# devincody/DSAbeamformer

Measured on AMD Instinct MI355X. Metric: beam-blocks/sec (256 beams x 256 freq x N_TIME), higher is better.
Workload: dtype int8 (int32 accumulate, fp32 detect)

## Files before the change

dsabeamformer_amd/api.py:

```python
from __future__ import annotations

import ctypes as C

from ._lib import BF_CAL_FULL, BF_CAL_PHASE, BfCalOptions, BfCondOptions, BfConfig, BfSkOptions, DsabfError, BfSpsCandidate, BfSpsPeak, BfSpsStat, check, load


def debug_config(**over) -> BfConfig:
    cfg = BfConfig()
    check(load().bf_config_default(C.byref(cfg), 1))
    for k, v in over.items():
        setattr(cfg, k, v)
    return cfg


def production_config(**over) -> BfConfig:
    cfg = BfConfig()
    check(load().bf_config_default(C.byref(cfg), 0))
    for k, v in over.items():
        setattr(cfg, k, v)
    return cfg


def launch_plan(cfg: BfConfig, paired: bool, n_units: int = 1, n_cus: int = 256) -> dict:
    g, b, l = C.c_int(), C.c_int(), C.c_int()
# ... 180 lines not shown
        check(self._lib.bf_stream_sync(self._h, stream_idx))

    def timer_start(self) -> None:
        check(self._lib.bf_timer_start(self._h))

    def timer_stop(self) -> float:
        ms = C.c_float()
        check(self._lib.bf_timer_stop(self._h, C.byref(ms)))
        return ms.value

    def mfma_peak(self, d_operands, operand_bytes: int, d_scratch, scratch_bytes: int, iters: int, stream) -> float:
        ops = C.c_double()
        check(self._lib.bf_mfma_peak_device(self._h, _ptr(d_operands), operand_bytes, _ptr(d_scratch), scratch_bytes, iters,
                                            C.byref(ops), C.c_void_p(stream)))
        return ops.value

    def gather_relayout(self, d_stage, d_full, rows_held: int, world: int, row_floats: int, skip_rank: int, stream: int = 0) -> None:
        check(self._lib.bf_gather_relayout_device(self._h, _ptr(d_stage), _ptr(d_full), rows_held, world, row_floats, skip_rank,
                                                  C.c_void_p(stream)))

    def set_switch(self, name: str, value: int) -> None:
        check(self._lib.bf_set_switch(self._h, name.encode(), int(value)))

    def counter(self, name: str) -> int:
        v = C.c_uint64()
        check(self._lib.bf_get_counter(self._h, name.encode(), C.byref(v)))
        return int(v.value)

    def kernel_info(self, n_units: int = 1) -> dict:
        g, b, l, v = C.c_int(), C.c_int(), C.c_int(), C.c_int()
        check(self._lib.bf_kernel_info(self._h, n_units, C.byref(g), C.byref(b), C.byref(l), C.byref(v)))
        name = C.create_string_buffer(160)
        check(self._lib.bf_kernel_name(self._h, name, 160))
        return {"kernel": name.value.decode(), "grid": g.value, "block": b.value, "lds_bytes": l.value,
                "vgprs": v.value}

    def variant_key(self, write_c: bool = False) -> str:
        buf = C.create_string_buffer(120)
        check(self._lib.bf_handle_variant_key(self._h, int(write_c), buf, 120))
        return buf.value.decode()


class DmStream(_Owner):
    _ptr_attr, _destroy = "_s", "bf_dm_stream_destroy"

    def __init__(self, bf: Beamformer, delays, n_freq_total: int, max_rows_per_push: int):
        import numpy as np

        self._lib = load()
        self._s = C.c_void_p()
        d = np.ascontiguousarray(delays, np.int32)
        assert d.ndim == 2 and d.shape[1] == n_freq_total
        self.n_dm, self.n_beams, self._bf = d.shape[0], bf.cfg.n_beams, bf
        check(self._lib.bf_dm_stream_create(bf._h, _ptr(d), d.shape[0], n_freq_total, max_rows_per_push, C.byref(self._s)))

    @property
    def max_delay(self) -> int:
        return self._lib.bf_dm_stream_max_delay(self._s)

    def push(self, d_rows, n_rows: int, host_out=None, stream: int = 0):
        first, n = C.c_uint64(), C.c_int()
        check(self._lib.bf_dm_stream_push(self._s, _ptr(d_rows), n_rows, _ptr(host_out), C.byref(first), C.byref(n), C.c_void_p(stream)))
        return int(first.value), int(n.value)

    def reserve(self, n_rows: int, stream: int = 0) -> int:
        p = C.c_void_p()
        check(self._lib.bf_dm_stream_reserve(self._s, n_rows, C.byref(p), C.c_void_p(stream)))
        return p.value or 0
# ... 342 lines not shown
```

dsabeamformer_amd/csrc/bf_bench_abi.cpp:

```cpp
#include "../../include/dsabf_bench.h"

#include <cstring>

#include "bf_runtime_internal.h"

extern "C" {

int bf_mfma_peak_device(bf_handle* h, const void* d_operands, size_t operand_bytes, void* d_scratch, size_t scratch_bytes, int iters,
                        double* ops, void* hip_stream)
{
    if (!h || !d_operands || !d_scratch) return fail(BF_ERR_INVALID, "NULL argument");
    if (operand_bytes < dsabf::kMfmaPeakSrcBytes || scratch_bytes < dsabf::kMfmaPeakSinkBytes || ((uintptr_t)d_operands & 15) || iters <= 0)
        return fail(BF_ERR_INVALID, "need >= %zu operand bytes (16-byte aligned), >= %zu scratch bytes, iters > 0",
                    dsabf::kMfmaPeakSrcBytes, dsabf::kMfmaPeakSinkBytes);
    ON_DEVICE(h);
    HIP_TRY(dsabf::launch_mfma_peak(d_operands, d_scratch, iters, h->n_cus, ops, as_stream(hip_stream)));
    return BF_OK;
}

int bf_gather_relayout_device(bf_handle* h, const float* d_stage, float* d_full, size_t rows_held, int world, size_t row_floats,
                              int skip_rank, void* hip_stream)
{
    if (!h || !d_stage || !d_full) return fail(BF_ERR_INVALID, "NULL argument");
    if (world < 1 || row_floats % 4 || ((uintptr_t)d_stage & 15) || ((uintptr_t)d_full & 15))
// ... 20 lines not shown
            FLUSH_UNITS(h);
            h->geom.fold = false;
        }
    } else if (!strcmp(name, "dm_wide")) {
        h->geom.dm_wide = value != 0;
    } else if (!strcmp(name, "coalesce")) {
        FLUSH_UNITS(h);
        h->coalesce = value != 0;
    } else if (!strcmp(name, "paired")) {
        h->force_general = value == 0;
    } else if (!strcmp(name, "fold")) {
        h->no_fold = value == 0;
    } else if (!strcmp(name, "dm_ring")) {
        h->dm_ring = value != 0;
    } else if (!strcmp(name, "cal_resident")) {
        h->cal_resident = value != 0;
    } else {
        return fail(BF_ERR_INVALID, "unknown switch \"%s\" (tsplit, rtw_kout, lds_pad, dm_wide, dm_ring, paired, fold, coalesce, cal_resident)", name);
    }
    return BF_OK;
}

int bf_get_counter(const bf_handle* h, const char* name, uint64_t* value)
{
    if (!h || !name || !value) return fail(BF_ERR_INVALID, "NULL argument");
    if (!strcmp(name, "fused_launches"))
        *value = h->n_fused_launches;
    else if (!strcmp(name, "queued_units"))
        *value = h->pending.size();
    else if (!strcmp(name, "dm_ring_stages")) {
        uint64_t n = 0;
        for (const bf_stage* s : h->stages) n += s->ring ? 1 : 0;
        *value = n;
    } else
        return fail(BF_ERR_INVALID, "unknown counter \"%s\" (fused_launches, queued_units, dm_ring_stages)", name);
    return BF_OK;
}

int bf_kernel_info(const bf_handle* h, int n_units, int* grid, int* block, int* lds_bytes, int* vgprs)
{
    if (!h) return fail(BF_ERR_INVALID, "handle is NULL");
    const dsabf::LaunchShape ls = dsabf::fused_launch_shape(h->geom, n_units > 0 ? n_units : 1, h->n_cus);
    if (grid) *grid = ls.grid;
    if (block) *block = ls.block;
    if (lds_bytes) *lds_bytes = ls.lds_bytes;
    if (vgprs) *vgprs = dsabf::fused_vgprs(h->geom);
    return BF_OK;
}

int bf_launch_plan(const bf_config* cfg, int paired, int n_units, int n_cus, int* grid, int* block, int* lds_bytes, char* name,
                   size_t name_len)
{
    dsabf::Geometry g{};
    if (int rc = supported_geom(cfg, g)) return rc;
    if (n_units <= 0 || n_cus <= 0) return fail(BF_ERR_INVALID, "need n_units > 0 and n_cus > 0");
    g.paired = paired && dsabf::pairing_supported(g);
    const dsabf::LaunchShape ls = dsabf::fused_launch_shape(g, n_units, n_cus);
    if (grid) *grid = ls.grid;
    if (block) *block = ls.block;
    if (lds_bytes) *lds_bytes = ls.lds_bytes;
    if (name && name_len) dsabf::fused_kernel_name(g, name, name_len);
    return BF_OK;
}

int bf_rtw_plan(const bf_config* cfg, int n_units, int n_cus, int* windows_per_stream, int* chunks_total)
{
    dsabf::Geometry g{};
    if (int rc = supported_geom(cfg, g)) return rc;
// ... 33 lines not shown
```

dsabeamformer_amd/csrc/bf_fused16.hpp:

```cpp
#pragma once
#include "bf_kernels.h"

#include <hip/hip_runtime.h>

#include <atomic>
#include <type_traits>

#ifndef DSABF_CLOCKPROBE
#define DSABF_CLOCKPROBE 0
#endif

namespace dsabf {

typedef int v4i __attribute__((ext_vector_type(4)));
typedef float v2f __attribute__((ext_vector_type(2)));
typedef float v4f __attribute__((ext_vector_type(4)));

constexpr int kDetCanonical = 0;
constexpr int kDetFast = 1;
constexpr int kDetContracted = 2;

constexpr int kAntK1P16 = -1;
constexpr int kAntK1P4 = -2;
constexpr int kAntK2P16 = -3;
// ... 76 lines not shown
{
    constexpr int LR = NIPO >= 32 ? 32 : 16;
    return chunk ^ ((((row >> 1) & 1) | (((row / LR) & 3) << 1)) ^ ((row & 1) << 2));
}

constexpr int kWaves16 = 4;
constexpr int kThreads16 = 64 * kWaves16;
constexpr int kWavesWide16 = 8;
constexpr int kColTiles16 = 4;
constexpr int kColTilesWide16 = 8;

template <int AIN>
constexpr int ant_ksteps()
{
    if (AIN > 0) return (AIN + 63) / 64;
    return (AIN == kAntK4P16 || AIN == kAntK4P4) ? 4 : (AIN == kAntK3P16 || AIN == kAntK3P4) ? 3 : (AIN == kAntK2P16 || AIN == kAntK2P4) ? 2 : 1;
}
template <int AIN>
constexpr bool ant_two_ksteps() { return ant_ksteps<AIN>() == 2; }
template <int AIN>
constexpr bool ant_deep() { return ant_ksteps<AIN>() > 2; }

template <int AIN, int NIPO, bool WRITE_C, int NS = kColTiles16>
constexpr int fused_min_waves()
{
    if (NS == 8 || ant_ksteps<AIN>() >= 2) return 2;
    if (AIN == kAntK1P16 && (NIPO == 8 || NIPO == 16 || NIPO == 32) && !WRITE_C) return 4;
    return 3;
}

template <int AIN, int NIPO, bool WRITE_C, int MODE = kDetCanonical, bool PAIRED = false, int WAVES = kWaves16, int NS = kColTiles16>
__global__ __launch_bounds__(64 * WAVES, (fused_min_waves<AIN, NIPO, WRITE_C, NS>())) void fused16_kernel(FusedArgs a)
{
    constexpr bool FOLD = false;
#include "bf_fused16_body.inc"
}

template <int NIPO>
struct FoldShape {
    static constexpr int AIN = kAntK1P16, WAVES = kWaves16, NS = kColTiles16;
    static constexpr bool WRITE_C = false, PAIRED = false;
};
template <int NIPO, int MODE>
__global__ __launch_bounds__(kThreads16, (fused_min_waves<kAntK1P16, NIPO, false>())) void fused16_fold_kernel(FusedArgs a)
{
    constexpr int AIN = FoldShape<NIPO>::AIN, WAVES = FoldShape<NIPO>::WAVES, NS = FoldShape<NIPO>::NS;
    constexpr bool WRITE_C = FoldShape<NIPO>::WRITE_C, PAIRED = FoldShape<NIPO>::PAIRED, FOLD = true;
#include "bf_fused16_body.inc"
}

template <int AIN, int NIPO, bool WRITE_C, int MODE, bool PAIRED, int WAVES, int NS>
hipError_t launch_fused16_t(const FusedArgs& args, const LaunchShape& ls, hipStream_t s)
{
    auto kern = fused16_kernel<AIN, NIPO, WRITE_C, MODE, PAIRED, WAVES, NS>;
    if (ls.block != 64 * WAVES || (args.interleave && args.interleave != (PAIRED ? NS / 2 : NS))) return hipErrorInvalidValue;
    if (ls.lds_bytes > 48 * 1024) {
        static std::atomic<unsigned> done_mask{0};
        int dev = 0;
        (void)hipGetDevice(&dev);
        const unsigned bit = 1u << (dev & 31);
        if (dev >= 32 || !(done_mask.load(std::memory_order_acquire) & bit)) {
            hipError_t e = hipFuncSetAttribute(reinterpret_cast<const void*>(kern), hipFuncAttributeMaxDynamicSharedMemorySize,
                                               ls.lds_bytes);
            if (e != hipSuccess) return e;
            done_mask.fetch_or(bit, std::memory_order_release);
        }
    }
    (void)hipGetLastError();
    hipLaunchKernelGGL(kern, dim3(ls.grid), dim3(ls.block), ls.lds_bytes, s, args);
    return hipGetLastError();
}

template <int NIPO, int MODE>
hipError_t launch_fused16_fold_t(const FusedArgs& args, const LaunchShape& ls, hipStream_t s)
{
    if (ls.block != kThreads16 || args.n_ant != 64 || (args.interleave && args.interleave != kColTiles16) || ls.lds_bytes > 48 * 1024)
        return hipErrorInvalidValue;
    (void)hipGetLastError();
    hipLaunchKernelGGL((fused16_fold_kernel<NIPO, MODE>), dim3(ls.grid), dim3(ls.block), ls.lds_bytes, s, args);
    return hipGetLastError();
}

using fused_launch_fn = hipError_t (*)(const FusedArgs&, const LaunchShape&, hipStream_t);
struct FusedVariant {
    const void* fn = nullptr;
    fused_launch_fn launch = nullptr;
    int ain = 0, nipo = 0, write_c = 0, mode = 0, paired = 0, waves = 0, ns = 0;
    int fold = 0;
};

template <int AIN, int NIPO, bool WRITE_C, int MODE, bool PAIRED, int WAVES, int NS = kColTiles16>
FusedVariant make_variant()
{
    return FusedVariant{reinterpret_cast<const void*>(fused16_kernel<AIN, NIPO, WRITE_C, MODE, PAIRED, WAVES, NS>),
                        launch_fused16_t<AIN, NIPO, WRITE_C, MODE, PAIRED, WAVES, NS>, AIN, NIPO, WRITE_C, MODE, PAIRED, WAVES, NS};
}

template <int AIN, int NIPO, int WAVES>
FusedVariant fused16_variant_nipo(bool write_c, int mode, bool paired)
{
    if (write_c) {
        if constexpr (WAVES == kWaves16) return make_variant<AIN, NIPO, true, kDetCanonical, false, WAVES>();
        return FusedVariant{};
    }
    if constexpr (NIPO >= 16 || NIPO == 0) {
        if (mode == kDetFast)
            return paired ? make_variant<AIN, NIPO, false, kDetFast, true, WAVES>() : make_variant<AIN, NIPO, false, kDetFast, false, WAVES>();
    }
    if (mode == kDetContracted)
        return paired ? make_variant<AIN, NIPO, false, kDetContracted, true, WAVES>()
                      : make_variant<AIN, NIPO, false, kDetContracted, false, WAVES>();
    return paired ? make_variant<AIN, NIPO, false, kDetCanonical, true, WAVES>() : make_variant<AIN, NIPO, false, kDetCanonical, false, WAVES>();
}

template <int AIN>
// ... 68 lines not shown
        if (mode == kDetFast) return make_variant<AIN, NIPO, false, kDetFast, true, kWavesWide16, 4>();
        if (mode == kDetContracted) return make_variant<AIN, NIPO, false, kDetContracted, true, kWavesWide16, 4>();
        return make_variant<AIN, NIPO, false, kDetCanonical, true, kWavesWide16, 4>();
    }
    if (mode == kDetFast) return make_variant<AIN, NIPO, false, kDetFast, false, kWavesWide16, 2>();
    if (mode == kDetContracted) return make_variant<AIN, NIPO, false, kDetContracted, false, kWavesWide16, 2>();
    return make_variant<AIN, NIPO, false, kDetCanonical, false, kWavesWide16, 2>();
}
template <int AIN>
FusedVariant fused16_variant_deep(int n_ipo, int mode, bool paired, int ns)
{
    static_assert(ant_deep<AIN>(), "three or four k-steps");
    switch (n_ipo) {
        case 16: return fused16_variant_deep_nipo<AIN, 16>(mode, paired, ns);
        case 32: return fused16_variant_deep_nipo<AIN, 32>(mode, paired, ns);
        case 64:
            if constexpr (AIN == kAntK3P4 || AIN == kAntK4P4) return FusedVariant{};
            else return fused16_variant_deep_nipo<AIN, 64>(mode, paired, ns);
        default: return FusedVariant{};
    }
}
FusedVariant fused16_variant_k4p16(int n_ipo, int mode, bool paired, int ns);
FusedVariant fused16_variant_k3p16(int n_ipo, int mode, bool paired, int ns);
FusedVariant fused16_variant_k4p4(int n_ipo, int mode, bool paired, int ns);
FusedVariant fused16_variant_k3p4(int n_ipo, int mode, bool paired, int ns);

template <int NIPO, int MODE>
FusedVariant make_fold_variant()
{
    return FusedVariant{reinterpret_cast<const void*>(fused16_fold_kernel<NIPO, MODE>), launch_fused16_fold_t<NIPO, MODE>, kAntK1P16, NIPO, 0, MODE,
                        0, kWaves16, kColTiles16, 1};
}
FusedVariant fused16_variant_k1p16_fold(int n_ipo, int mode);

FusedVariant fused16_variant_a100(int n_ipo, bool write_c, int mode, bool paired);
FusedVariant fused16_variant_k1p16(int n_ipo, bool write_c, int mode, bool paired);
FusedVariant fused16_variant_k1p4(int n_ipo, bool write_c, int mode, bool paired);
FusedVariant fused16_variant_k2p16(int n_ipo, bool write_c, int mode, bool paired);
FusedVariant fused16_variant_k2p4(int n_ipo, bool write_c, int mode, bool paired);
FusedVariant fused16_variant_a100_w8(int n_ipo, int mode);
FusedVariant fused16_variant_k2p16_w8(int n_ipo, int mode);
FusedVariant fused16_variant_k2p4_w8(int n_ipo, int mode);
FusedVariant fused16_variant_a100_w8p(int n_ipo, int mode);
FusedVariant fused16_variant_k2p16_w8p(int n_ipo, int mode);
FusedVariant fused16_variant_k2p4_w8p(int n_ipo, int mode);
FusedVariant fused16_variant_a100_s8(int n_ipo, int mode);
FusedVariant fused16_variant_k2p16_s8(int n_ipo, int mode);
FusedVariant fused16_variant_k2p4_s8(int n_ipo, int mode);

}
```

dsabeamformer_amd/csrc/bf_fused16_body.inc:

```
    constexpr int THREADS = 64 * WAVES;
    constexpr bool FAST = MODE == kDetFast;
    constexpr bool CONTRACTED = MODE == kDetContracted;
    constexpr bool RTW = NIPO == 0;
    constexpr int MAPN = RTW ? 32 : NIPO;
    static_assert(!FAST || ((NIPO >= 16 || RTW) && !WRITE_C), "the fast detect exists for n_ipo >= 16 only");
    static_assert(!RTW || (WAVES == kWaves16 && NS == kColTiles16 && !ant_deep<AIN>()), "run-time windows: the plain launch shape");
    static_assert(!(PAIRED && WRITE_C), "the stage-parity path always runs the general kernel");
    static_assert(AIN >= kAntK3P4 && AIN != 0 && (AIN < 0 || AIN % 4 == 0) && AIN <= 256, "antenna class");
    static_assert(!ant_deep<AIN>() || (WAVES == 8 && NIPO >= 16 && !WRITE_C), "deep classes: 8 waves, long windows");
    static_assert(!FOLD || (AIN == kAntK1P16 && NIPO >= 16 && !WRITE_C && !PAIRED && WAVES == kWaves16 && NS == kColTiles16),
                  "antenna fold: 64 antennas in 16-byte pieces, long compile-time windows, general tiles on the plain launch shape");
    constexpr bool OFFSET_NIB = ant_deep<AIN>();
    constexpr float kA = FOLD ? kAlpha8 : OFFSET_NIB ? kAlpha : kAlpha16;
    constexpr float kNKA = FOLD ? kNegMagicAlpha8 : OFFSET_NIB ? kNegMagicAlpha : kNegMagicAlpha16;
    constexpr bool RT = AIN < 0;
    constexpr int RB = 128;
    constexpr int KS = ant_ksteps<AIN>();
    constexpr int PLANE = kRowsPerChunk * RB;
    constexpr int BUF = KS * PLANE;
    constexpr bool DW = RT ? (AIN == kAntK1P4 || AIN == kAntK2P4 || AIN == kAntK3P4 || AIN == kAntK4P4) : (AIN % 16) != 0;
    constexpr int PB = DW ? 4 : 16;
    constexpr int AMAX = RT ? 64 * KS : AIN;
    const int A = FOLD ? 64 : RT ? a.n_ant : AIN;
    const int PPR = A / PB;
    const int TOTALP = kRowsPerChunk * PPR;
    constexpr int TOTALP_MAX = kRowsPerChunk * (AMAX / PB);
    constexpr int NT = PAIRED ? NS / 2 : NS;
    constexpr bool LONG = NIPO >= 16;
    constexpr int L = LONG ? NIPO : 16;
    constexpr int LR = (NIPO >= 32 || RTW) ? 32 : 16;
    constexpr int CPG = L > 32 ? L / 32 : 1;
    constexpr int PPT = (TOTALP_MAX + THREADS - 1) / THREADS;
    using stage_t = std::conditional_t<DW, int, v4i>;

    extern __shared__ __attribute__((aligned(16))) char smem[];

    const int tid = threadIdx.x;
    const int lane = tid & 63;
    const int wave = __builtin_amdgcn_readfirstlane(tid >> 6);
    const int g4 = lane >> 4;
    const int c16 = lane & 15;

    int f, bg, ts;
    decode_block(a, f, bg, ts);
// ... 58 lines not shown
            sacc += __shfl_xor(sacc, 32);
            return sacc;
        };
#pragma unroll
        for (int t = 0; t < NT; t++) {
            int s0, s1;
            if constexpr (PAIRED) {
                s0 = (int)kMagicBits - 8 * colsum(bw[t][0]);
                s1 = -8 * colsum(bw[t][1]);
            } else {
                const int wr = colsum(bw[t][0]), nwi = colsum(bw[t][1]), wi = colsum(bw[t][2]);
                s0 = (int)kMagicBits - 8 * (wr + nwi);
                s1 = (int)kMagicBits - 8 * (wi + wr);
            }
            sd[t][0] = v4i{s0, s0, s0, s0};
            sd[t][1] = v4i{s1, s1, s1, s1};
            asm volatile("" : "+v"(sd[t][0]), "+v"(sd[t][1]));
        }
    }

    auto run_sample0 = [&](int c, int run) -> unsigned {
        if constexpr (RTW)
            return (4u * (unsigned)(c / cpg_rt) + (unsigned)run) * (unsigned)a.rt_Ls + 32u * (unsigned)(c % cpg_rt);
        else if constexpr (NIPO >= 32)
            return (4u * (unsigned)(c / CPG) + (unsigned)run) * (unsigned)L + 32u * (unsigned)(c % CPG);
        else
            return (unsigned)c * 128u + 16u * (unsigned)run;
    };
    stage_t stage[PPT];
    constexpr unsigned SPAN = (NIPO == 64) ? 256u : 128u;
    const bool fast_addr = !RTW && ((unsigned)a.T % SPAN) == 0;
    [[maybe_unused]] unsigned lane_off64[NIPO == 64 ? PPT : 1];
    int lds_re[PPT];
#pragma unroll
    for (int k = 0; k < PPT; k++) {
        int row, pi;
        if constexpr (FOLD) {
            row = tid >> 1;
            pi = k == 0 ? (tid & 1) : 3 - (tid & 1);
        } else {
            const int pc = tid + k * THREADS;
            row = (pc / PPR) % kRowsPerChunk, pi = pc % PPR;
        }
        if constexpr (NIPO == 64) lane_off64[k] = (unsigned)((row / LR) * L + (row % LR)) * A + pi * PB;
        const int blk = DW ? pi / 4 : pi;
        const int h = blk / 4, kp = blk % 4, sub = DW ? 4 * (pi % 4) : 0;
        lds_re[k] = h * PLANE + row * RB + 16 * swz16<MAPN>(kp + 4 * (h & 1), row) + sub;
    }
    auto lane_off = [&](int k) -> unsigned {
        if constexpr (NIPO == 64)
            return lane_off64[k];
        else if constexpr (FOLD)
            return (unsigned)(64 * (tid >> 1) + 16 * (k == 0 ? (tid & 1) : 3 - (tid & 1)));
        else
            return (unsigned)PB * (unsigned)(tid + k * THREADS);
    };
    auto piece_live = [&](int k) { return (!RT && TOTALP_MAX % THREADS == 0) || (tid + k * THREADS < TOTALP); };
    int ld_span = -1;
    unsigned ld_u = 0, ld_t0 = 0;
    auto load_chunk = [&](int c) {
        if (fast_addr) {
            const int span = (NIPO == 64) ? c / 2 : c;
            if (ld_span < 0) {
                const unsigned s_c = (unsigned)span * SPAN;
                ld_u = a.t_shift >= 0 ? (s_c >> a.t_shift) : (s_c / (unsigned)a.T);
                ld_t0 = s_c - ld_u * (unsigned)a.T;
                ld_span = span;
            }
            while (ld_span < span) {
                ld_t0 += SPAN;
                if (ld_t0 >= (unsigned)a.T) {
                    ld_t0 = 0;
                    ld_u++;
                }
                ld_span++;
            }
            const bool valid = (unsigned)span * SPAN < a.S;
            const unsigned half = (NIPO == 64) ? 32u * (unsigned)(c & 1) : 0u;
            const uint8_t* base = a.in + ((size_t)((size_t)ld_u * a.n_freq + f) * a.T + ld_t0 + half) * A;
#pragma unroll
            for (int k = 0; k < PPT; k++) {
                stage[k] = stage_t{};
                if (valid && piece_live(k)) stage[k] = *reinterpret_cast<const stage_t*>(base + lane_off(k));
            }
            return;
        }
#pragma unroll
        for (int k = 0; k < PPT; k++) {
            int row, pi;
            if constexpr (FOLD) {
                row = tid >> 1;
                pi = k == 0 ? (tid & 1) : 3 - (tid & 1);
            } else {
                const int pc = tid + k * THREADS;
                row = (pc / PPR) % kRowsPerChunk, pi = pc % PPR;
            }
            const unsigned s0 = run_sample0(c, row / LR) + (unsigned)(row % LR);
            stage[k] = stage_t{};
            bool row_ok = s0 < a.S;
            if constexpr (RTW) row_ok = row_ok && 32u * (unsigned)(c % cpg_rt) + (unsigned)(row % LR) < (unsigned)a.rt_Ls;
            if (row_ok && piece_live(k)) {
                const unsigned u = a.t_shift >= 0 ? (s0 >> a.t_shift) : (s0 / (unsigned)a.T);
                const unsigned t = s0 - u * (unsigned)a.T;
                stage[k] = *reinterpret_cast<const stage_t*>(a.in + ((size_t)((size_t)u * a.n_freq + f) * a.T + t) * A + pi * PB);
            }
        }
    };
    auto write_chunk = [&](char* buf) {
        if constexpr (FOLD) {
            constexpr unsigned M = 0x78787878u, H = 0x80808080u;
            v4i sr, si, dr, di;
#pragma unroll
            for (int d = 0; d < 4; d++) {
                const unsigned ta = (unsigned)stage[0][d] ^ 0x88888888u;
                const unsigned tb = __builtin_bswap32((unsigned)stage[PPT - 1][3 - d]) ^ 0x88888888u;
                const unsigned ra = (ta >> 1) & M, ia = (ta << 3) & M, rb = (tb >> 1) & M, ib = (tb << 3) & M;
                sr[d] = (int)((ra + rb) ^ H);
                si[d] = (int)((ia + ib) ^ H);
                dr[d] = (int)(((ra | H) - rb) ^ H);
                di[d] = (int)(((ia | H) - ib) ^ H);
            }
            *reinterpret_cast<v4i*>(buf + lds_re[0]) = sr;
            *reinterpret_cast<v4i*>(buf + (lds_re[0] ^ 32)) = di;
            *reinterpret_cast<v4i*>(buf + (lds_re[0] ^ 64)) = dr;
            *reinterpret_cast<v4i*>(buf + (lds_re[0] ^ 96)) = si;
            return;
        }
#pragma unroll
        for (int k = 0; k < PPT; k++) {
            if (!piece_live(k)) continue;
            if constexpr (DW) {
                const unsigned w = (unsigned)stage[k];
                if constexpr (OFFSET_NIB) {
                    const unsigned x = w ^ 0x88888888u;
                    *reinterpret_cast<int*>(buf + lds_re[k]) = (int)((x >> 4) & 0x0F0F0F0Fu);
                    *reinterpret_cast<int*>(buf + (lds_re[k] ^ 64)) = (int)(x & 0x0F0F0F0Fu);
                } else {
                    *reinterpret_cast<int*>(buf + lds_re[k]) = (int)(w & 0xF0F0F0F0u);
                    *reinterpret_cast<int*>(buf + (lds_re[k] ^ 64)) = (int)((w << 4) & 0xF0F0F0F0u);
                }
            } else {
                v4i re, im;
#pragma unroll
// ... 25 lines not shown
    for (int gi = 0; gi < PEND; gi++) pend_chunk[gi] = -1;
    auto store_slots = [&](float* row, const float (&x)[NS]) {
        if (a.interleave) {
            if constexpr (PAIRED && NS == 2) {
                row[slot_beam[0]] = x[0];
                row[slot_beam[1]] = x[1];
            } else if constexpr (PAIRED && NS == 4) {
                __builtin_nontemporal_store(v2f{x[0], x[2]}, reinterpret_cast<v2f*>(row + slot_beam[0]));
                __builtin_nontemporal_store(v2f{x[3], x[1]}, reinterpret_cast<v2f*>(row + slot_beam[3]));
            } else if constexpr (PAIRED) {
                __builtin_nontemporal_store(v4f{x[0], x[2], x[4], x[6]}, reinterpret_cast<v4f*>(row + slot_beam[0]));
                __builtin_nontemporal_store(v4f{x[7], x[5], x[3], x[1]}, reinterpret_cast<v4f*>(row + slot_beam[7]));
            } else if constexpr (NS == 2) {
                __builtin_nontemporal_store(v2f{x[0], x[1]}, reinterpret_cast<v2f*>(row + slot_beam[0]));
            } else {
#pragma unroll
                for (int q = 0; q < NS; q += 4)
                    __builtin_nontemporal_store(v4f{x[q], x[q + 1], x[q + 2], x[q + 3]}, reinterpret_cast<v4f*>(row + slot_beam[q]));
            }
        } else {
#pragma unroll
            for (int sl = 0; sl < NS; sl++)
                if (slot_beam[sl] < a.n_beams) row[slot_beam[sl]] = x[sl];
        }
    };
    auto flush_pending = [&]() {
        if constexpr (LONG && !WRITE_C) {
#pragma unroll
            for (int gi = 0; gi < PEND; gi++) {
                if (pend_chunk[gi] >= 0 && wave_active) {
                    const unsigned grp = (NIPO >= 32) ? (unsigned)(pend_chunk[gi] / CPG) : (2u * pend_chunk[gi] + gi);
                    float* ub = a.out + ((size_t)(4u * grp) * FB + (size_t)f * a.n_beams);
                    const unsigned o = 4u * grp + (unsigned)g4;
                    if (o * (unsigned)L < a.S) store_slots(ub + (size_t)g4 * FB, pend[gi]);
                }
                pend_chunk[gi] = -1;
            }
        }
    };

    if (c_begin >= c_end) return;
#if DSABF_CLOCKPROBE
    const unsigned long long probe_t0 = __builtin_amdgcn_s_memtime(), probe_r0 = __builtin_amdgcn_s_memrealtime();
#endif

    load_chunk(c_begin);
    write_chunk(smem);
    if (c_begin + 1 < c_end) load_chunk(c_begin + 1);
    __syncthreads();

    const bool stage_only = FOLD && !wave_active;
    if (stage_only)
        for (int c = c_begin; c < c_end; c++) {
            if (c + 1 < c_end) write_chunk(smem + ((c - c_begin + 1) & 1) * BUF);
            if (c + 2 < c_end) load_chunk(c + 2);
            __syncthreads();
        }
    for (int c = stage_only ? c_end : c_begin; c < c_end; c++) {
        char* cur = smem + ((c - c_begin) & 1) * BUF;
        char* nxt = smem + ((c - c_begin + 1) & 1) * BUF;
        if (!FOLD && !wave_active) {
            if (c + 1 < c_end) write_chunk(nxt);
            if (c + 2 < c_end) load_chunk(c + 2);
        } else {
            [[maybe_unused]] float ov[2][NS];
            [[maybe_unused]] bool rt_st[4] = {false, false, false, false}, rt_en[4] = {false, false, false, false};
            [[maybe_unused]] unsigned rt_o[4] = {0, 0, 0, 0};
            [[maybe_unused]] float rt_x[4][NS];
            [[maybe_unused]] int rt_m = 0;
            [[maybe_unused]] unsigned rt_oq = 0;
            if constexpr (RTW) {
                const unsigned p0 = 32u * (unsigned)(c % cpg_rt);
                rt_m = (int)(p0 % (unsigned)a.rt_L);
                rt_oq = p0 / (unsigned)a.rt_L;
            }
            auto detect = [&](const int t8, const v4f fr, const v4f fi, const int sl) {
                const int gi = (NIPO >= 32) ? 0 : (t8 >> 2);
                const int q4 = (NIPO >= 32) ? (32 * (c % CPG) + 4 * t8) : 4 * (t8 & 3);
                const unsigned grp = (NIPO >= 32) ? (unsigned)(c / CPG) : (2u * (unsigned)c + gi);
                const unsigned o = 4u * grp + (unsigned)g4;
                const int beam = slot_beam[sl];
                if constexpr (WRITE_C && RTW) {
#pragma unroll
                    for (int r = 0; r < 4; r++) {
                        const unsigned pos = 32u * (unsigned)(c % cpg_rt) + 4u * t8 + r;
                        const unsigned sidx = (4u * (unsigned)(c / cpg_rt) + (unsigned)g4) * (unsigned)a.rt_Ls + pos;
                        if (pos < (unsigned)a.rt_Ls && sidx < a.S && beam < a.n_beams) {
                            v2f cv = {__builtin_fmaf(fr[r], kA, kNKA), __builtin_fmaf(fi[r], kA, kNKA)};
// ... 121 lines not shown
            auto dot = [&](const v4i (&x)[KS], const v4i (&w)[KS], v4i acc) {
#pragma unroll
                for (int h = 0; h < KS; h++) acc = __builtin_amdgcn_mfma_i32_16x16x64_i8(x[h], w[h], acc, 0, 0, 0);
                return acc;
            };
            constexpr int SPS = PAIRED ? 2 : 1;
            auto issue = [&](const v4i (&a0)[KS], const v4i (&a1)[KS], const int t, v4i (&re)[SPS], v4i (&im)[SPS]) {
                const v4i k0 = OFFSET_NIB ? sd[OFFSET_NIB ? t : 0][0] : kc;
                const v4i k1 = OFFSET_NIB ? sd[OFFSET_NIB ? t : 0][1] : (PAIRED ? kzero : kc);
                if constexpr (PAIRED) {
                    const v4i p1 = dot(a0, bw[t][0], k0);
                    const v4i p3 = dot(a1, bw[t][0], k0);
                    const v4i p2 = dot(a1, bw[t][1], k1);
                    const v4i p4 = dot(a0, bw[t][1], k1);
                    re[0] = p1 - p2;
                    re[1] = p1 + p2;
                    im[0] = p3 + p4;
                    im[1] = p3 - p4;
                } else if constexpr (FOLD) {
                    re[0] = dot(a0, bw[t][0], k0);
                    im[0] = dot(a1, bw[t][NGC - 1], k1);
                } else {
                    re[0] = dot(a1, bw[t][1], dot(a0, bw[t][0], k0));
                    im[0] = dot(a1, bw[t][0], dot(a0, bw[t][2], k1));
                }
            };
            auto consume = [&](const int t8, const int t, const v4i (&re)[SPS], const v4i (&im)[SPS]) {
#pragma unroll
                for (int e = 0; e < SPS; e++) {
                    detect(t8, __builtin_bit_cast(v4f, re[e]), __builtin_bit_cast(v4f, im[e]), SPS * t + e);
                }
            };
            auto staging = [&](const int t8) {
                if (t8 == 1 && c + 1 < c_end) write_chunk(nxt);
                if (t8 == 3) {
                    flush_pending();
                    if (c + 2 < c_end) load_chunk(c + 2);
                }
            };
#pragma unroll
            for (int t8 = 0; t8 < 8; t8++) {
                v4i a0[KS], a1[KS];
                read_frag(t8, a0, a1);
                if constexpr (RTW) {
#pragma unroll
                    for (int r = 0; r < 4; r++) {
                        rt_st[r] = rt_m == 0;
                        rt_en[r] = ++rt_m == a.rt_L;
                        if (rt_en[r]) {
                            rt_m = 0;
                            rt_o[r] = rt_oq++;
                            rt_en[r] = rt_o[r] < (unsigned)a.rt_kout;
                        }
                    }
                }
#pragma unroll
                for (int t = 0; t < NT; t++) {
                    v4i re[SPS], im[SPS];
                    issue(a0, a1, t, re, im);
                    consume(t8, t, re, im);
                }
                if constexpr (RTW && !WRITE_C) {
                    const unsigned sigma = 4u * (unsigned)(c / cpg_rt) + (unsigned)g4;
#pragma unroll
                    for (int r = 0; r < 4; r++)
                        if (rt_en[r]) {
                            const unsigned o = sigma * (unsigned)a.rt_kout + rt_o[r];
                            if ((unsigned long long)o * (unsigned)a.rt_L < a.S) store_slots(a.out + (size_t)o * FB + (size_t)f * a.n_beams, rt_x[r]);
                        }
                }
// ... 15 lines not shown
```

dsabeamformer_amd/csrc/bf_kernels.h:

```cpp
#pragma once

#include <hip/hip_runtime.h>
#include <stddef.h>
#include <stdint.h>

namespace dsabf {

constexpr int kRowsPerChunk = 128;

struct Geometry {
    int n_beams, n_ant, n_freq, n_ipo, n_out, n_time;
    int n_ctiles;
    bool fast_detect;
    bool contracted_detect = false;
    bool paired = false;
    bool fold = false;
    bool plain_wg_waves = false;
    bool plain_col_tiles = false;
    int rtw_kout = 0;
    int tsplit = 0;
    int lds_pad = 0;
    bool dm_wide = true;
    bool force_generic = false;
    bool no_rtw = false;
    bool no_deep = false;
};
constexpr int kLdsPerCuBytes = 160 * 1024;
void read_env_switches(Geometry& g);
bool lab_mode();
const char* lab_getenv(const char* name);

size_t weight_image_bytes(const Geometry& g);

bool pairing_supported(const Geometry& g);
size_t weight_pair_image_bytes(const Geometry& g);
bool fold_supported(const Geometry& g);
size_t weight_fold_image_bytes(const Geometry& g);

bool fused_supported(const Geometry& g, const char** why);

struct LaunchShape {
    int grid, block, lds_bytes, n_tsplit, chunks_total;
    int rt_kout;
    int n_bgroups;
};
int fused_wg_waves(const Geometry& g, bool write_c = false);
int fused_col_tiles(const Geometry& g, bool paired);
LaunchShape fused_launch_shape(const Geometry& g, int n_units, int n_cus, bool write_c = false);
int rtw_kout(const Geometry& g, long long S, long long base, int n_cus);

hipError_t launch_weight_relayout(const Geometry& g, const int8_t* d_w, void* d_image, void* d_pair_image, void* d_fold_image,
                                  int* d_bad, hipStream_t s);

hipError_t launch_fused(const Geometry& g, const void* d_image, const void* d_pair_image, const void* d_fold_image, const void* d_packed,
                        int n_units, float* d_out, int n_cus, hipStream_t s);

hipError_t launch_gemm_only(const Geometry& g, const void* d_image, const void* d_packed, float* d_c, int n_cus,
                            hipStream_t s);

hipError_t launch_expand(const void* d_in, size_t nbytes, void* d_out, hipStream_t s);
constexpr size_t kMfmaPeakSrcBytes = (size_t)(512 + 256) * 256 * 16;
constexpr size_t kMfmaPeakSinkBytes = (size_t)4096 * 256 * sizeof(int);
hipError_t launch_mfma_peak(const void* d_src, void* d_sink, int iters, int n_cus, double* ops, hipStream_t s);
hipError_t launch_gather_relayout(const float* d_stage, float* d_full, size_t held, int world, size_t row_floats, int skip_rank,
                                  int n_cus, hipStream_t s);
hipError_t launch_dedisperse(const Geometry& g, const float* d_out_unit, float* d_ded, hipStream_t s);
hipError_t launch_dedisperse_units(const Geometry& g, const float* d_out_units, size_t unit_stride, int n_units, float* d_ded,
                                   hipStream_t s);
hipError_t launch_dedisperse_dm(const Geometry& g, const float* d_series, int n_t, const int* d_delays, int n_dm,
                                int n_t_out, float* d_out, int* d_flags, hipStream_t s);
// ... 28 lines not shown
```

dsabeamformer_amd/csrc/bf_kernels.hip:

```cpp
#include "bf_fused16.hpp"

#include <cstdio>
#include <cstdlib>

namespace dsabf {

namespace {

__device__ __forceinline__ unsigned sext4x4(unsigned nib)
{
    return ((nib ^ 0x88888888u) - 0x08080808u) ^ 0x80808080u;
}

typedef int v2i_t __attribute__((ext_vector_type(2)));

__global__ __launch_bounds__(256) void expand_kernel(const v2i_t* __restrict__ in, v4i* __restrict__ out, size_t n_half)
{
    const size_t wave = ((size_t)blockIdx.x * blockDim.x + threadIdx.x) / 64, n_waves = (size_t)gridDim.x * blockDim.x / 64;
    const int lane = threadIdx.x & 63;
    for (size_t base = wave * 128; base < n_half; base += n_waves * 128) {
#pragma unroll
        for (int p = 0; p < 2; p++) {
            const size_t i = base + p * 64 + lane;
            if (i >= n_half) break;
// ... 290 lines not shown
                if (wi == -128) *bad = 1;
                v = (comp == 1) ? -wi : (comp == 2) ? wi : wr;
            }
            d[i >> 2] |= ((unsigned)v & 0xFFu) << (8 * (i & 3));
        }
        image[idx] = v4i{(int)d[0], (int)d[1], (int)d[2], (int)d[3]};
    }
}


int ksteps16(const Geometry& g) { return (g.n_ant + 63) / 64; }
bool deep_class(const Geometry& g)
{
    return !g.force_generic && !g.no_deep && g.n_ant > 128 && g.n_ant <= 256 && g.n_ant % 4 == 0 &&
           (g.n_ipo == 16 || g.n_ipo == 32 || (g.n_ipo == 64 && g.n_ant % 16 == 0));
}
int interleaved(const Geometry& g, bool paired)
{
    if (use_generic(g)) return paired ? 0 : generic_interleave(g);
    const int ns = fused_col_tiles(g, paired);
    if (g.n_beams % (16 * ns)) return 0;
    return paired ? ns / 2 : ns;
}
bool nipo_supported(int n_ipo) { return n_ipo == 2 || n_ipo == 4 || n_ipo == 8 || n_ipo == 16 || n_ipo == 32 || n_ipo == 64; }
bool rtw_class(const Geometry& g)
{
    return !g.force_generic && !g.no_rtw && g.n_ant <= 128 && g.n_ipo > 0 && (!nipo_supported(g.n_ipo) || (g.n_ipo < 16 && g.n_time % 16));
}
int detect_mode_of(const Geometry& g) { return g.fast_detect ? kDetFast : g.contracted_detect ? kDetContracted : kDetCanonical; }

FusedVariant select_variant(const Geometry& g, bool write_c)
{
    if (use_generic(g)) return FusedVariant{};
    if (g.fold && !write_c) return fused16_variant_k1p16_fold(g.n_ipo, detect_mode_of(g));
    if (deep_class(g)) {
        if (write_c) return FusedVariant{};
        const bool paired = g.paired;
        const int mode = detect_mode_of(g);
        const int ns = fused_col_tiles(g, paired);
        if (g.n_ant % 16) return g.n_ant > 192 ? fused16_variant_k4p4(g.n_ipo, mode, paired, ns) : fused16_variant_k3p4(g.n_ipo, mode, paired, ns);
        return g.n_ant > 192 ? fused16_variant_k4p16(g.n_ipo, mode, paired, ns) : fused16_variant_k3p16(g.n_ipo, mode, paired, ns);
    }
    if ((!nipo_supported(g.n_ipo) && !rtw_class(g)) || g.n_ant <= 0 || g.n_ant > 128 || g.n_ant % 4) return FusedVariant{};
    const bool paired = g.paired && !write_c;
    const int sel_ipo = rtw_class(g) ? 0 : g.n_ipo;
    const int mode = (detect_mode_of(g) == kDetFast && g.n_ipo < 16) ? kDetCanonical : detect_mode_of(g);
    if (fused_col_tiles(g, paired) == kColTilesWide16) {
        if (g.n_ant == 100) return fused16_variant_a100_s8(g.n_ipo, mode);
        return g.n_ant % 16 == 0 ? fused16_variant_k2p16_s8(g.n_ipo, mode) : fused16_variant_k2p4_s8(g.n_ipo, mode);
    }
    if (fused_wg_waves(g, write_c) == kWavesWide16) {
        if (paired) {
            if (g.n_ant == 100) return fused16_variant_a100_w8p(g.n_ipo, mode);
            return g.n_ant % 16 == 0 ? fused16_variant_k2p16_w8p(g.n_ipo, mode) : fused16_variant_k2p4_w8p(g.n_ipo, mode);
        }
        if (g.n_ant == 100) return fused16_variant_a100_w8(g.n_ipo, mode);
        return g.n_ant % 16 == 0 ? fused16_variant_k2p16_w8(g.n_ipo, mode) : fused16_variant_k2p4_w8(g.n_ipo, mode);
    }
    if (g.n_ant == 100) return fused16_variant_a100(sel_ipo, write_c, mode, paired);
    if (g.n_ant <= 64)
        return g.n_ant % 16 == 0 ? fused16_variant_k1p16(sel_ipo, write_c, mode, paired) : fused16_variant_k1p4(sel_ipo, write_c, mode, paired);
    return g.n_ant % 16 == 0 ? fused16_variant_k2p16(sel_ipo, write_c, mode, paired) : fused16_variant_k2p4(sel_ipo, write_c, mode, paired);
}

int ilog2_exact(int v)
{
    if (v <= 0 || (v & (v - 1))) return -1;
// ... 5 lines not shown
hipError_t dispatch_fused(const Geometry& g, bool write_c, const FusedArgs& args, const LaunchShape& ls, hipStream_t s)
{
    const FusedVariant v = select_variant(g, write_c);
    if (!v.launch) return hipErrorInvalidValue;
    return v.launch(args, ls, s);
}

}

bool use_generic(const Geometry& g)
{
    if (g.force_generic || (g.n_ant > 128 && !deep_class(g))) return true;
    return (!nipo_supported(g.n_ipo) || (g.n_ipo < 16 && g.n_time % 16)) && !rtw_class(g);
}

size_t weight_image_bytes(const Geometry& g)
{
    return (size_t)g.n_freq * g.n_ctiles * kGeneralComps * ksteps16(g) * 64 * 16 +
           ((use_generic(g) || deep_class(g)) ? generic_image_extra_bytes(g) : 0);
}

bool pairing_supported(const Geometry& g)
{
    return !use_generic(g) && g.n_beams % 32 == 0 && select_variant(g, false).launch != nullptr;
}
size_t weight_pair_image_bytes(const Geometry& g)
{
    return pairing_supported(g) ? (size_t)g.n_freq * (g.n_beams / 32) * kPairComps * ksteps16(g) * 64 * 16 : 0;
}

bool fold_supported(const Geometry& g)
{
    return !use_generic(g) && !deep_class(g) && !rtw_class(g) && g.n_ant == 64 && (g.n_ipo == 16 || g.n_ipo == 32 || g.n_ipo == 64);
}
size_t weight_fold_image_bytes(const Geometry& g)
{
    return fold_supported(g) ? (size_t)g.n_freq * g.n_ctiles * kFoldComps * 64 * 16 : 0;
}

bool fused_supported(const Geometry& g, const char** why)
{
    const char* dummy;
    if (!why) why = &dummy;
    if (g.n_beams <= 0 || g.n_beams % 4) { *why = "N_BEAMS must be a positive multiple of 4"; return false; }
    if (g.n_ant <= 0 || g.n_ant % 4) { *why = "N_ANTENNAS must be a positive multiple of 4"; return false; }
    if (use_generic(g)) return generic_supported(g, why);
    return true;
}

bool lab_mode()
{
    const char* lab = getenv("DSABF_LAB");
    return lab && lab[0] == '1' && !lab[1];
}
const char* lab_getenv(const char* name) { return lab_mode() ? getenv(name) : nullptr; }

void read_env_switches(Geometry& g)
{
    const char* w = lab_getenv("DSABF_WG_WAVES");
    const char* t = lab_getenv("DSABF_COL_TILES");
    g.plain_wg_waves = w && atoi(w) == kWaves16;
    g.plain_col_tiles = t && atoi(t) == kColTiles16;
    const char* ts = lab_getenv("DSABF_TSPLIT");
    const char* pad = lab_getenv("DSABF_LDS_PAD");
    const char* dw = lab_getenv("DSABF_DM_WIDE");
    g.tsplit = ts ? atoi(ts) : 0;
// ... 345 lines not shown
```

Before: 2.356 million.

## Add streamed fold kernel with incremental SGPR base addressing and permuted row mapping

Adds a fused16_fold_stream_kernel variant, chosen when fold is active and n_time divides the span. It replaces per-chunk address computation with a running scalar base pointer advanced in the chunk loop, plus precomputed per-lane offsets. It also permutes the row-to-thread mapping and drops tail bounds checks on stores. The aim is to cut integer address arithmetic and branch overhead in the staging path, in exchange for an explicit waitcnt before LDS writes and one extra kernel instantiation.

```diff
diff --git a/dsabeamformer_amd/api.py b/dsabeamformer_amd/api.py
--- a/dsabeamformer_amd/api.py
+++ b/dsabeamformer_amd/api.py
@@ -236,8 +236,14 @@
         check(self._lib.bf_kernel_info(self._h, n_units, C.byref(g), C.byref(b), C.byref(l), C.byref(v)))
         name = C.create_string_buffer(160)
         check(self._lib.bf_kernel_name(self._h, name, 160))
+        key = self.variant_key()
+        launch = key.split("<")[0]
+        if launch == "fused16_fold_kernel":
+            v64 = C.c_uint64()
+            if self._lib.bf_get_counter(self._h, b"fold_stream", C.byref(v64)) == 0 and v64.value:
+                launch = "fused16_fold_stream_kernel"
         return {"kernel": name.value.decode(), "grid": g.value, "block": b.value, "lds_bytes": l.value,
-                "vgprs": v.value}
+                "vgprs": v.value, "launch": launch}
 
     def variant_key(self, write_c: bool = False) -> str:
         buf = C.create_string_buffer(120)
diff --git a/dsabeamformer_amd/csrc/bf_bench_abi.cpp b/dsabeamformer_amd/csrc/bf_bench_abi.cpp
--- a/dsabeamformer_amd/csrc/bf_bench_abi.cpp
+++ b/dsabeamformer_amd/csrc/bf_bench_abi.cpp
@@ -76,8 +76,10 @@
         uint64_t n = 0;
         for (const bf_stage* s : h->stages) n += s->ring ? 1 : 0;
         *value = n;
-    } else
-        return fail(BF_ERR_INVALID, "unknown counter \"%s\" (fused_launches, queued_units, dm_ring_stages)", name);
+    } else if (!strcmp(name, "fold_stream"))
+        *value = dsabf::fold_streams(h->geom) ? 1 : 0;
+    else
+        return fail(BF_ERR_INVALID, "unknown counter \"%s\" (fused_launches, queued_units, dm_ring_stages, fold_stream)", name);
     return BF_OK;
 }
 
diff --git a/dsabeamformer_amd/csrc/bf_fused16.hpp b/dsabeamformer_amd/csrc/bf_fused16.hpp
--- a/dsabeamformer_amd/csrc/bf_fused16.hpp
+++ b/dsabeamformer_amd/csrc/bf_fused16.hpp
@@ -132,7 +132,7 @@
 template <int AIN, int NIPO, bool WRITE_C, int MODE = kDetCanonical, bool PAIRED = false, int WAVES = kWaves16, int NS = kColTiles16>
 __global__ __launch_bounds__(64 * WAVES, (fused_min_waves<AIN, NIPO, WRITE_C, NS>())) void fused16_kernel(FusedArgs a)
 {
-    constexpr bool FOLD = false;
+    constexpr bool FOLD = false, STREAM = false;
 #include "bf_fused16_body.inc"
 }
 
@@ -145,7 +145,17 @@
 __global__ __launch_bounds__(kThreads16, (fused_min_waves<kAntK1P16, NIPO, false>())) void fused16_fold_kernel(FusedArgs a)
 {
     constexpr int AIN = FoldShape<NIPO>::AIN, WAVES = FoldShape<NIPO>::WAVES, NS = FoldShape<NIPO>::NS;
-    constexpr bool WRITE_C = FoldShape<NIPO>::WRITE_C, PAIRED = FoldShape<NIPO>::PAIRED, FOLD = true;
+    constexpr bool WRITE_C = FoldShape<NIPO>::WRITE_C, PAIRED = FoldShape<NIPO>::PAIRED, FOLD = true, STREAM = false;
+#include "bf_fused16_body.inc"
+}
+
+template <int NIPO>
+constexpr unsigned fold_stream_span() { return NIPO == 64 ? 256u : 128u; }
+template <int NIPO, int MODE>
+__global__ __launch_bounds__(kThreads16, (fused_min_waves<kAntK1P16, NIPO, false>())) void fused16_fold_stream_kernel(FusedArgs a)
+{
+    constexpr int AIN = FoldShape<NIPO>::AIN, WAVES = FoldShape<NIPO>::WAVES, NS = FoldShape<NIPO>::NS;
+    constexpr bool WRITE_C = FoldShape<NIPO>::WRITE_C, PAIRED = FoldShape<NIPO>::PAIRED, FOLD = true, STREAM = true;
 #include "bf_fused16_body.inc"
 }
 
@@ -181,6 +191,19 @@
     return hipGetLastError();
 }
 
+template <int NIPO, int MODE>
+hipError_t launch_fused16_fold_stream_t(const FusedArgs& args, const LaunchShape& ls, hipStream_t s)
+{
+    if (ls.block != kThreads16 || args.n_ant != 64 || (args.interleave && args.interleave != kColTiles16) || ls.lds_bytes > 48 * 1024)
+        return hipErrorInvalidValue;
+    if (args.T <= 0 || (unsigned)args.T % fold_stream_span<NIPO>() != 0 || args.chunks_total <= 0 ||
+        (unsigned long long)args.chunks_total * kRowsPerChunk != args.S)
+        return hipErrorInvalidValue;
+    (void)hipGetLastError();
+    hipLaunchKernelGGL((fused16_fold_stream_kernel<NIPO, MODE>), dim3(ls.grid), dim3(ls.block), ls.lds_bytes, s, args);
+    return hipGetLastError();
+}
+
 using fused_launch_fn = hipError_t (*)(const FusedArgs&, const LaunchShape&, hipStream_t);
 struct FusedVariant {
     const void* fn = nullptr;
@@ -315,6 +338,14 @@
                         0, kWaves16, kColTiles16, 1};
 }
 FusedVariant fused16_variant_k1p16_fold(int n_ipo, int mode);
+
+template <int NIPO, int MODE>
+FusedVariant make_fold_stream_variant()
+{
+    return FusedVariant{reinterpret_cast<const void*>(fused16_fold_stream_kernel<NIPO, MODE>), launch_fused16_fold_stream_t<NIPO, MODE>, kAntK1P16,
+                        NIPO, 0, MODE, 0, kWaves16, kColTiles16, 2};
+}
+FusedVariant fused16_variant_k1p16_fold_stream(int n_ipo, int mode);
 
 FusedVariant fused16_variant_a100(int n_ipo, bool write_c, int mode, bool paired);
 FusedVariant fused16_variant_k1p16(int n_ipo, bool write_c, int mode, bool paired);
diff --git a/dsabeamformer_amd/csrc/bf_fused16_body.inc b/dsabeamformer_amd/csrc/bf_fused16_body.inc
--- a/dsabeamformer_amd/csrc/bf_fused16_body.inc
+++ b/dsabeamformer_amd/csrc/bf_fused16_body.inc
@@ -10,6 +10,7 @@
     static_assert(!ant_deep<AIN>() || (WAVES == 8 && NIPO >= 16 && !WRITE_C), "deep classes: 8 waves, long windows");
     static_assert(!FOLD || (AIN == kAntK1P16 && NIPO >= 16 && !WRITE_C && !PAIRED && WAVES == kWaves16 && NS == kColTiles16),
                   "antenna fold: 64 antennas in 16-byte pieces, long compile-time windows, general tiles on the plain launch shape");
+    static_assert(!STREAM || FOLD, "the streamed chunk loop exists for the antenna-fold kernels");
     constexpr bool OFFSET_NIB = ant_deep<AIN>();
     constexpr float kA = FOLD ? kAlpha8 : OFFSET_NIB ? kAlpha : kAlpha16;
     constexpr float kNKA = FOLD ? kNegMagicAlpha8 : OFFSET_NIB ? kNegMagicAlpha : kNegMagicAlpha16;
@@ -134,11 +135,18 @@
     const bool fast_addr = !RTW && ((unsigned)a.T % SPAN) == 0;
     [[maybe_unused]] unsigned lane_off64[NIPO == 64 ? PPT : 1];
     int lds_re[PPT];
+    [[maybe_unused]] const int fold_row = [&] {
+        const int q = tid >> 1;
+        if constexpr (!STREAM) return q;
+        else if constexpr (LR == 32) return (q & 1) | (((q >> 1) & 3) << 5) | (((q >> 3) & 15) << 1);
+        else return (q & 1) | (((q >> 1) & 3) << 4) | (((q >> 3) & 7) << 1) | ((q >> 6) << 6);
+    }();
 #pragma unroll
     for (int k = 0; k < PPT; k++) {
         int row, pi;
         if constexpr (FOLD) {
-            row = tid >> 1;
+            if constexpr (STREAM) row = fold_row;
+            else row = tid >> 1;
             pi = k == 0 ? (tid & 1) : 3 - (tid & 1);
         } else {
             const int pc = tid + k * THREADS;
@@ -152,6 +160,8 @@
     auto lane_off = [&](int k) -> unsigned {
         if constexpr (NIPO == 64)
             return lane_off64[k];
+        else if constexpr (STREAM)
+            return (unsigned)(64 * fold_row + 16 * (k == 0 ? (tid & 1) : 3 - (tid & 1)));
         else if constexpr (FOLD)
             return (unsigned)(64 * (tid >> 1) + 16 * (k == 0 ? (tid & 1) : 3 - (tid & 1)));
         else
@@ -208,9 +218,59 @@
             }
         }
     };
+    [[maybe_unused]] unsigned long long st_base = 0;
+    [[maybe_unused]] unsigned st_t0 = 0;
+    [[maybe_unused]] int st_next = c_begin;
+    [[maybe_unused]] unsigned long long st_unit = 0;
+    [[maybe_unused]] unsigned st_off[PPT];
+    if constexpr (STREAM) {
+        const unsigned s_c = (unsigned)(NIPO == 64 ? c_begin / 2 : c_begin) * SPAN;
+        const unsigned u = a.t_shift >= 0 ? (s_c >> a.t_shift) : (s_c / (unsigned)a.T);
+        st_t0 = s_c - u * (unsigned)a.T;
+        auto sgpr64 = [](unsigned long long v) {
+            return (unsigned long long)(unsigned)__builtin_amdgcn_readfirstlane((int)(unsigned)v) |
+                   ((unsigned long long)(unsigned)__builtin_amdgcn_readfirstlane((int)(unsigned)(v >> 32)) << 32);
+        };
+        st_base = sgpr64((unsigned long long)((size_t)((size_t)u * a.n_freq + f) * a.T + st_t0) * 64);
+        st_t0 = (unsigned)__builtin_amdgcn_readfirstlane((int)st_t0);
+        st_unit = sgpr64((unsigned long long)(unsigned)(a.n_freq - 1) * (unsigned)a.T * 64);
+#pragma unroll
+        for (int k = 0; k < PPT; k++) st_off[k] = lane_off(k);
+    }
+    auto load_stream = [&]() {
+        unsigned long long base = (unsigned long long)a.in + st_base;
+        asm volatile("" : "+s"(base));
+#pragma unroll
+        for (int k = 0; k < PPT; k++) {
+            unsigned off = st_off[k];
+            asm volatile("" : "+v"(off));
+            stage[k] = *(const __attribute__((address_space(1))) stage_t*)(base + off);
+        }
+        if (st_next + 1 < c_end) {
+            bool next_span = true;
+            if constexpr (NIPO == 64) {
+                next_span = (st_next & 1) != 0;
+                st_base += next_span ? (size_t)(SPAN - 32u) * 64 : (size_t)32 * 64;
+            } else {
+                st_base += (size_t)SPAN * 64;
+            }
+            if (next_span) {
+                st_t0 += SPAN;
+                if (st_t0 >= (unsigned)a.T) {
+                    st_t0 = 0;
+                    st_base += st_unit;
+                }
+            }
+            st_next++;
+        }
+    };
     auto write_chunk = [&](char* buf) {
         if constexpr (FOLD) {
             constexpr unsigned M = 0x78787878u, H = 0x80808080u;
+            if constexpr (STREAM) {
+                __builtin_amdgcn_s_waitcnt(0x0F70);
+                asm volatile("" : "+v"(stage[0]), "+v"(stage[PPT - 1]));
+            }
             v4i sr, si, dr, di;
 #pragma unroll
             for (int d = 0; d < 4; d++) {
@@ -302,7 +362,7 @@
                     const unsigned grp = (NIPO >= 32) ? (unsigned)(pend_chunk[gi] / CPG) : (2u * pend_chunk[gi] + gi);
                     float* ub = a.out + ((size_t)(4u * grp) * FB + (size_t)f * a.n_beams);
                     const unsigned o = 4u * grp + (unsigned)g4;
-                    if (o * (unsigned)L < a.S) store_slots(ub + (size_t)g4 * FB, pend[gi]);
+                    if (STREAM || o * (unsigned)L < a.S) store_slots(ub + (size_t)g4 * FB, pend[gi]);
                 }
                 pend_chunk[gi] = -1;
             }
@@ -314,16 +374,27 @@
     const unsigned long long probe_t0 = __builtin_amdgcn_s_memtime(), probe_r0 = __builtin_amdgcn_s_memrealtime();
 #endif
 
-    load_chunk(c_begin);
-    write_chunk(smem);
-    if (c_begin + 1 < c_end) load_chunk(c_begin + 1);
+    if constexpr (STREAM) {
+        load_stream();
+        write_chunk(smem);
+        load_stream();
+    } else {
+        load_chunk(c_begin);
+        write_chunk(smem);
+        if (c_begin + 1 < c_end) load_chunk(c_begin + 1);
+    }
     __syncthreads();
 
     const bool stage_only = FOLD && !wave_active;
     if (stage_only)
         for (int c = c_begin; c < c_end; c++) {
-            if (c + 1 < c_end) write_chunk(smem + ((c - c_begin + 1) & 1) * BUF);
-            if (c + 2 < c_end) load_chunk(c + 2);
+            if constexpr (STREAM) {
+                write_chunk(smem + ((c - c_begin + 1) & 1) * BUF);
+                load_stream();
+            } else {
+                if (c + 1 < c_end) write_chunk(smem + ((c - c_begin + 1) & 1) * BUF);
+                if (c + 2 < c_end) load_chunk(c + 2);
+            }
             __syncthreads();
         }
     for (int c = stage_only ? c_end : c_begin; c < c_end; c++) {
@@ -511,10 +582,18 @@
                 }
             };
             auto staging = [&](const int t8) {
-                if (t8 == 1 && c + 1 < c_end) write_chunk(nxt);
-                if (t8 == 3) {
-                    flush_pending();
-                    if (c + 2 < c_end) load_chunk(c + 2);
+                if constexpr (STREAM) {
+                    if (t8 == 1) write_chunk(nxt);
+                    if (t8 == 3) {
+                        load_stream();
+                        flush_pending();
+                    }
+                } else {
+                    if (t8 == 1 && c + 1 < c_end) write_chunk(nxt);
+                    if (t8 == 3) {
+                        flush_pending();
+                        if (c + 2 < c_end) load_chunk(c + 2);
+                    }
                 }
             };
 #pragma unroll
diff --git a/dsabeamformer_amd/csrc/bf_fused16_k1p16_fold_stream.hip b/dsabeamformer_amd/csrc/bf_fused16_k1p16_fold_stream.hip
--- /dev/null
+++ b/dsabeamformer_amd/csrc/bf_fused16_k1p16_fold_stream.hip
@@ -0,0 +1,23 @@
+#include "bf_fused16.hpp"
+
+namespace dsabf {
+namespace {
+template <int NIPO>
+FusedVariant fold_stream_nipo(int mode)
+{
+    if (mode == kDetFast) return make_fold_stream_variant<NIPO, kDetFast>();
+    if (mode == kDetContracted) return make_fold_stream_variant<NIPO, kDetContracted>();
+    return make_fold_stream_variant<NIPO, kDetCanonical>();
+}
+}
+
+FusedVariant fused16_variant_k1p16_fold_stream(int n_ipo, int mode)
+{
+    switch (n_ipo) {
+        case 16: return fold_stream_nipo<16>(mode);
+        case 32: return fold_stream_nipo<32>(mode);
+        case 64: return fold_stream_nipo<64>(mode);
+        default: return FusedVariant{};
+    }
+}
+}
diff --git a/dsabeamformer_amd/csrc/bf_kernels.h b/dsabeamformer_amd/csrc/bf_kernels.h
--- a/dsabeamformer_amd/csrc/bf_kernels.h
+++ b/dsabeamformer_amd/csrc/bf_kernels.h
@@ -36,6 +36,7 @@
 size_t weight_pair_image_bytes(const Geometry& g);
 bool fold_supported(const Geometry& g);
 size_t weight_fold_image_bytes(const Geometry& g);
+bool fold_streams(const Geometry& g);
 
 bool fused_supported(const Geometry& g, const char** why);
 
diff --git a/dsabeamformer_amd/csrc/bf_kernels.hip b/dsabeamformer_amd/csrc/bf_kernels.hip
--- a/dsabeamformer_amd/csrc/bf_kernels.hip
+++ b/dsabeamformer_amd/csrc/bf_kernels.hip
@@ -346,7 +346,8 @@
 FusedVariant select_variant(const Geometry& g, bool write_c)
 {
     if (use_generic(g)) return FusedVariant{};
-    if (g.fold && !write_c) return fused16_variant_k1p16_fold(g.n_ipo, detect_mode_of(g));
+    if (g.fold && !write_c)
+        return fold_streams(g) ? fused16_variant_k1p16_fold_stream(g.n_ipo, detect_mode_of(g)) : fused16_variant_k1p16_fold(g.n_ipo, detect_mode_of(g));
     if (deep_class(g)) {
         if (write_c) return FusedVariant{};
         const bool paired = g.paired;
@@ -418,6 +419,10 @@
 bool fold_supported(const Geometry& g)
 {
     return !use_generic(g) && !deep_class(g) && !rtw_class(g) && g.n_ant == 64 && (g.n_ipo == 16 || g.n_ipo == 32 || g.n_ipo == 64);
+}
+bool fold_streams(const Geometry& g)
+{
+    return g.fold && fold_supported(g) && g.n_time > 0 && g.n_time % (g.n_ipo == 64 ? 256 : 128) == 0;
 }
 size_t weight_fold_image_bytes(const Geometry& g)
 {
```

Measured after the change: 2.423 million, median of 6. +2.9%, better.
